# ebiggers/libdeflate

Hardware: NVIDIA H100
Metric: MB/s compress+decompress (batched 64 KiB chunks) (higher is better)
Workload: dtype u8

## Files before the change

### libdeflate_b200/csrc/deflate_lz_kernel.cuh

```cuda
#pragma once

#define LZ_THREADS   1024
#define LZ_WARPS     (LZ_THREADS / 32)
#define LZ_PASS      16384
#define LZ_BLOCK_PASSES 2
#define LZ_NWIN      (LZ_PASS / 32)
#define LZ_NSL_BITS  5
#define LZ_NSL       (1 << LZ_NSL_BITS)
#define LZ_SEG       16384
#define LZ_RING      65536
#define LZ_HASH_BITS 13
#define LZ_WIN       32768
#define LZ_LOOKAHEAD 512
#define LZ_MAX_DIST  (LZ_WIN - LZ_LOOKAHEAD)
#define LZ_TOKCAP    (LZ_BLOCK_PASSES * LZ_PASS + 64)
#define LZ_STAGE_WORDS 2048
#define LZ_TPT(gt)     ((gt) > 512 ? 1u : 2u)
#define LZ_GROUP_PARSE     {12, 10, 8, 8, 8, 5, 16, 16, 16}
#define LZ_GROUP_FLUSH     12
#define LZ_GROUP_HAND      10
#define LZ_GROUP_MIN_PARSE 4
#define LZ_GROUP_MIN_FLUSH 10
#define LZ_GROUP_MAX       28
#define LZ_BAR_P     1
#define LZ_BAR_S     2
#define LZ_BAR_H     3
#define LZ_PF        4
#define LZ_RUN_SHORT 16
#ifndef LZ_SPEC_ROUNDS
#define LZ_SPEC_ROUNDS 4
#endif
static_assert(LZ_SPEC_ROUNDS >= 1 && LZ_SPEC_ROUNDS <= 14, "round statistic buckets");
static_assert(LZ_GROUP_MIN_PARSE >= 1 && LZ_GROUP_MIN_FLUSH * 32 >= 320 && LZ_GROUP_MAX < LZ_WARPS, "group size bounds");
static_assert(LZ_GROUP_FLUSH >= LZ_GROUP_MIN_FLUSH && LZ_GROUP_FLUSH <= LZ_GROUP_MAX && LZ_GROUP_HAND >= LZ_GROUP_MIN_FLUSH &&
	      LZ_GROUP_HAND <= LZ_GROUP_MAX, "default group sizes");

#define LZ_SM_RING   0
#define LZ_SM_NEXT   (LZ_SM_RING + LZ_RING)
#define LZ_SM_HEAD   (LZ_SM_NEXT + 2 * 65536)
#define LZ_SM_R      (LZ_SM_HEAD + 2 * (1 << LZ_HASH_BITS))
#define LZ_SM_VIS    (LZ_SM_R)
#define LZ_SM_TOKOFF (LZ_SM_R + 4096)
#define LZ_SM_ENTRY  (LZ_SM_R + 8320)
#define LZ_SM_ESCAN  (LZ_SM_R + 9344)
#define LZ_SM_GEXIT  (LZ_SM_R + 9728)
#define LZ_SM_ITEMS  (LZ_SM_R + 12288)
#define LZ_SM_FREQ   (LZ_SM_ITEMS + 1024)
#define LZ_SM_LENS   (LZ_SM_FREQ + 4 * 320)
#define LZ_SM_CODES  (LZ_SM_LENS + 320)
#define LZ_SM_VARS   (LZ_SM_CODES + 2 * 320)
#define LZ_SM_BYTES  (LZ_SM_VARS + 256)

#define LZ_BLOCK_POS (LZ_BLOCK_PASSES * LZ_PASS)
#define LZ_OPT_K     8
#define LZ_DP_SEG    2048
#define LZ_GS_RES    0
#define LZ_GS_TOK    (LZ_GS_RES + 4 * LZ_BLOCK_POS)
#define LZ_GS_COST   (LZ_GS_TOK + 4 * LZ_TOKCAP)
#define LZ_GS_MLIST  (LZ_GS_COST + 4 * (LZ_BLOCK_POS + 320))
#define LZ_GS_BYTES  (LZ_GS_MLIST + 4 * LZ_BLOCK_POS * LZ_OPT_K)
#define LZ_FAR4_DIST  1024
#define LZ_COST_INF  0x3fffffu

struct lz_vars {
	unsigned long long mbar;
	u32 chunk;
	u32 tok_count;
	u32 parse_entry;
	u32 cost_dyn, cost_static;
	u32 hlit, hdist, hclen;
	u32 n_items;
	u32 run_counter;
	u32 min_len;
	u32 far4_dist;
	u32 used_lits[8];
	u32 carry;
	u32 nused_lit, nused_off;
	u32 huff_over;
	u32 obs_blk[8], obs_next[8];
	u32 end_block;
	u32 failed;
	u32 obit_lo, obit_hi;
	u32 blk_begin, blk_entry, blk_passes;
	u32 pre_lens_packed[3];
	u32 tma_phase;
	u32 dict, nonfinal;
	u32 spec_last;
	u32 spec_first;
	u32 prefetched;
	u32 nx_min_len, nx_far4;
};
static_assert(sizeof(lz_vars) <= 256, "lz_vars fits its shared-memory slot");

struct lz_params {
	int depth, nice, lazy;
	int opt_iters;
};

__device__ __forceinline__ lz_params lz_level_params(int level)
{
	switch (level) {
	case 1: return {2, 16, 0, 0};
	case 2: return {4, 24, 0, 0};
	case 3: return {8, 32, 0, 0};
	case 4: return {12, 48, 0, 0};
	case 5: return {12, 48, 1, 0};
	case 6: return {24, 96, 1, 0};
	case 7: return {48, 160, 1, 0};
	case 8: return {96, 258, 2, 0};
	case 9: return {200, 258, 2, 0};
	case 10: return {48, 96, 1, 2};
	case 11: return {96, 160, 1, 3};
	default: return {200, 258, 1, 5};
	}
}

__device__ __forceinline__ u32 lz_choose_min_len(u32 num_used_literals, u32 depth)
{
	u32 m;
	if (num_used_literals < 6) m = 9;
	else if (num_used_literals < 8) m = 8;
	else if (num_used_literals < 10) m = 7;
	else if (num_used_literals < 16) m = 6;
	else if (num_used_literals < 45) m = 5;
	else m = 4;
	if (depth < 16) {
		u32 cap = depth < 5 ? 4 : (depth < 10 ? 5 : 7);
		if (m > cap) m = cap;
	}
	return m;
}

__device__ __forceinline__ u32 lz_ld32(const u8 *ring, u32 pos)
{
	u32 a = pos & (LZ_RING - 1);
	const u32 *w = (const u32 *)ring;
	u32 lo = w[a >> 2];
	u32 hi = w[((a + 4) & (LZ_RING - 1)) >> 2];
	return __funnelshift_r(lo, hi, (a & 3) * 8);
}
__device__ __forceinline__ u32 lz_ld8(const u8 *ring, u32 pos) { return ring[pos & (LZ_RING - 1)]; }
__device__ __forceinline__ u32 lz_hash(u32 v) { return (v * 0x1E35A7BDu) >> (32 - LZ_HASH_BITS); }

__device__ __forceinline__ u32 lz_len_slot(u32 len)
{
	if (len < 11) return len - 3;
	if (len == 258) return 28;
	u32 l = len - 3;
	u32 eb = 29 - __clz(l);
	return 4 * eb + 4 + ((l >> eb) & 3);
}
__device__ __forceinline__ u32 lz_len_extra_bits(u32 slot) { return (slot < 8 || slot == 28) ? 0 : (slot - 4) >> 2; }
__device__ __forceinline__ u32 lz_len_base(u32 slot) { return slot < 8 ? 3 + slot : (slot == 28 ? 258 : 3 + ((4 + (slot & 3)) << ((slot - 4) >> 2))); }
__device__ __forceinline__ u32 lz_off_slot(u32 off)
{
	if (off < 5) return off - 1;
	u32 o = off - 1;
	u32 eb = 30 - __clz(o);
	return 2 * eb + 2 + ((o >> eb) & 1);
}
__device__ __forceinline__ u32 lz_off_extra_bits(u32 slot) { return slot < 4 ? 0 : (slot - 2) >> 1; }
__device__ __forceinline__ u32 lz_off_base(u32 slot) { return slot < 4 ? 1 + slot : 1 + ((2 + (slot & 1)) << ((slot - 2) >> 1)); }

#include "deflate_block.cuh"

__device__ __forceinline__ void lz_load_segment(const lz_group &g, u8 *sm, const u8 *in, u32 from, u32 to)
{
	u8 *ring = sm + LZ_SM_RING;
	lz_vars *v = (lz_vars *)(sm + LZ_SM_VARS);
	u32 len = to - from;
	u32 bulk = (((uintptr_t)(in + from) & 15) == 0) ? (len & ~15u) : 0;
	g.sync();
#ifndef LDB_EMU
	if (bulk) {
		u32 mbar = (u32)__cvta_generic_to_shared(&v->mbar);
		if (g.tid == 0) {
			u32 dst = (u32)__cvta_generic_to_shared(ring + (from & (LZ_RING - 1)));
			asm volatile("fence.proxy.async.shared::cta;" ::: "memory");
			asm volatile("mbarrier.arrive.expect_tx.shared::cta.b64 _, [%0], %1;" ::"r"(mbar), "r"(bulk) : "memory");
			asm volatile("cp.async.bulk.shared::cluster.global.mbarrier::complete_tx::bytes [%0], [%1], %2, [%3];"
				     ::"r"(dst), "l"(in + from), "r"(bulk), "r"(mbar) : "memory");
		}
		u32 phase = v->tma_phase;
		u32 done = 0;
		while (!done) {
			asm volatile("{\n\t.reg .pred p;\n\tmbarrier.try_wait.parity.shared::cta.b64 p, [%1], %2;\n\tselp.u32 %0, 1, 0, p;\n\t}"
				     : "=r"(done) : "r"(mbar), "r"(phase) : "memory");
		}
	}
#else
	for (u32 i = g.tid; i < bulk; i += g.gt) ring[(from + i) & (LZ_RING - 1)] = in[from + i];
#endif
	for (u32 i = bulk + g.tid; i < len; i += g.gt) ring[(from + i) & (LZ_RING - 1)] = in[from + i];
	g.sync();
	if (bulk && g.tid == 0) v->tma_phase ^= 1;
	g.sync();
}

#ifdef LZ_TIMING
#include <stdio.h>
#define LZ_TSLOTS 30
__device__ unsigned long long ldb_lz_timing[2][LZ_TSLOTS];
struct lz_clock {
	bool on, t0;
	long long tacc[LZ_TSLOTS] = {}, tlast = 0, tspan = 0, tsplit = 0, tbusy = 0, tjoin = 0;
	__device__ explicit lz_clock(u32 tid)
	{
		on = tid == 0 || tid == LZ_THREADS - 32;
		t0 = tid == 0;
		tlast = clock64();
	}
	__device__ void mark(int k) { if (on) { const long long t = clock64(); tacc[k] += t - tlast; tlast = t; } }
	__device__ void span_begin() { if (on) tspan = clock64(); }
	__device__ void span_end(int k) { if (on) tacc[k] += clock64() - tspan; }
	__device__ void split_begin() { if (on) tsplit = clock64(); }
	__device__ void split_busy() { if (t0) tbusy = clock64() - tsplit; }
	__device__ void join_begin() { if (on) tjoin = clock64(); }
	__device__ void split_end(bool split, int kind)
	{
		if (!split || !on) return;
		const long long t = clock64();
		tacc[18 + kind] += tbusy; tacc[21 + kind] += t - tjoin; tacc[24 + kind] += 1; tacc[27 + kind] += t - tsplit;
	}
	__device__ void commit() const
	{
		if (on)
			for (int k = 0; k < LZ_TSLOTS; k++) atomicAdd(&ldb_lz_timing[t0 ? 0 : 1][k], (unsigned long long)tacc[k]);
	}
};
#else
struct lz_clock {
	__device__ explicit lz_clock(u32) {}
	__device__ __forceinline__ void mark(int) {}
	__device__ __forceinline__ void span_begin() {}
	__device__ __forceinline__ void span_end(int) {}
	__device__ __forceinline__ void split_begin() {}
	__device__ __forceinline__ void split_busy() {}
	__device__ __forceinline__ void join_begin() {}
	__device__ __forceinline__ void split_end(bool, int) {}
	__device__ __forceinline__ void commit() const {}
};
#endif

#ifdef LZ_SPEC_STATS
__device__ unsigned long long ldb_lz_spec_rounds[16];
extern "C" __attribute__((visibility("default"))) void ldb_lz_spec_stats(unsigned long long *out, int reset)
{
#ifdef LDB_EMU
	for (int i = 0; i < 16; i++) { out[i] = ldb_lz_spec_rounds[i]; if (reset) ldb_lz_spec_rounds[i] = 0; }
#else
	unsigned long long z[16] = {};
	cudaDeviceSynchronize();
	cudaMemcpyFromSymbol(out, ldb_lz_spec_rounds, sizeof(z));
	if (reset) cudaMemcpyToSymbol(ldb_lz_spec_rounds, z, sizeof(z));
#endif
}
#endif

template <int NBITS>
__device__ __forceinline__ u32 lz_same_key_mask(u32 key, bool valid)
{
	u32 m = __ballot_sync(LDB_FULL_MASK, valid);
#pragma unroll
	for (int b = 0; b < NBITS; b++) {
		const u32 bal = __ballot_sync(LDB_FULL_MASK, (key >> b) & 1);
		m &= ((key >> b) & 1) ? bal : ~bal;
	}
	return m;
}

template <typename Decided>
__device__ __forceinline__ void lz_insert_pass_par(const lz_group &g, u8 *sm, u32 *cmat, u32 b0, u32 pend, u32 n,
						   bool decide, Decided decided, lz_clock &clk)
{
	const u8 *ring = sm + LZ_SM_RING;
	u16 *head = (u16 *)(sm + LZ_SM_HEAD);
	u16 *nextt = (u16 *)(sm + LZ_SM_NEXT);
	const u32 tid = g.tid, lane = g.lane, warp = g.warp, gw = g.gw;
	static_assert((LZ_WARPS * LZ_NSL + 2 * LZ_NSL) * 4 <= 8192, "count matrix fits the start of region R");
	u32 *sbase = cmat + LZ_WARPS * LZ_NSL, *stot = sbase + LZ_NSL;
	const u32 lt = (1u << lane) - 1;
	const u32 LB = (b0 + LZ_PASS) & 0xffff;
	const u32 ntiles = (pend - b0 + 31) >> 5, tpw = (ntiles + gw - 1) / gw;
	const u32 r0 = b0 + warp * tpw * 32;
	const u32 r1 = r0 + tpw * 32 < pend ? r0 + tpw * 32 : pend;
	for (u32 i = tid; i < LZ_WARPS * LZ_NSL + 2 * LZ_NSL; i += 32 * gw) cmat[i] = 0;
	g.sync();
	for (u32 p = r0 + lane; p < r1; p += 32) {
		const u32 hv = p + 4 <= n ? lz_hash(lz_ld32(ring, p)) : 0xffffu;
		nextt[p & 0xffff] = (u16)hv;
		if (hv != 0xffffu) atomicAdd(&cmat[warp * LZ_NSL + (hv >> (LZ_HASH_BITS - LZ_NSL_BITS))], 1u);
	}
	g.sync();
	clk.mark(12);
	if (decide && tid == 32 * (gw - 1)) decided();
	if (warp == 0) {
		u32 run = 0;
		if (lane < LZ_NSL)
			for (u32 w = 0; w < gw; w++) {
				const u32 c = cmat[w * LZ_NSL + lane];
				cmat[w * LZ_NSL + lane] = run;
				run += c;
			}
		u32 incl = run;
		for (int o2 = 1; o2 < LZ_NSL; o2 <<= 1) {
			const u32 t = __shfl_up_sync(LDB_FULL_MASK, incl, o2);
			if (lane >= (u32)o2) incl += t;
		}
		if (lane < LZ_NSL) { sbase[lane] = incl - run; stot[lane] = run; }
	}
	g.sync();
	for (u32 t = 0; t < tpw; t++) {
		const u32 p = r0 + 32 * t + lane;
		const u32 hv = p < r1 ? nextt[p & 0xffff] : 0xffffu;
		const bool valid = hv != 0xffffu;
		const u32 sl = hv >> (LZ_HASH_BITS - LZ_NSL_BITS);
		const u32 m = lz_same_key_mask<LZ_NSL_BITS>(sl, valid);
		const u32 cur = valid ? cmat[warp * LZ_NSL + sl] : 0;
		__syncwarp();
		if (valid) {
			nextt[LB + sbase[sl] + cur + __popc(m & lt)] = (u16)p;
			if ((m & lt) == 0) cmat[warp * LZ_NSL + sl] = cur + __popc(m);
		}
		__syncwarp();
	}
	g.sync();
	clk.mark(13);
	for (u32 s = warp; s < LZ_NSL; s += gw) {
		const u32 cnt = stot[s];
		const u16 *mylist = nextt + LB + sbase[s];
		u32 p16n = lane < cnt ? mylist[lane] : 0;
		u32 hn = lane < cnt ? nextt[p16n] : 0;
		for (u32 b = 0; b < cnt; b += 32) {
			const bool valid = b + lane < cnt;
			const u32 p16 = p16n;
			const u32 h = valid ? hn : 0;
			if (b + 32 + lane < cnt) {
				p16n = mylist[b + 32 + lane];
				hn = nextt[p16n];
			}
			const u32 old_head = valid ? head[h] : 0;
			const u32 m = lz_same_key_mask<LZ_HASH_BITS - LZ_NSL_BITS>(h, valid);
			const u32 below = m & lt;
			const u32 prev = __shfl_sync(LDB_FULL_MASK, p16, below ? 31 - __clz(below) : 0);
			if (valid) {
				nextt[p16] = (u16)(below ? prev : old_head);
				if ((m >> lane) == 1) head[h] = (u16)p16;
			}
			__syncwarp();
		}
	}
	g.sync();
}

__device__ __forceinline__ void lz_observe(const u8 *ring, u32 from, u32 to, u32 *obs, u32 tid, u32 lane, u32 nthreads)
{
	for (u32 wbase = from + 512 * (tid >> 5); wbase < to; wbase += 16 * nthreads) {
		const u32 base = wbase + 16 * lane;
		const uint4 q = *(const uint4 *)(ring + (base & (LZ_RING - 1)));
		const u32 w[4] = {q.x, q.y, q.z, q.w};
		u64 cnt = 0;
#pragma unroll
		for (int k = 0; k < 16; k++) {
			const u32 bv = (w[k >> 2] >> (8 * (k & 3))) & 0xff;
			if (base + k < to) cnt += (u64)1 << (8 * (((bv >> 5) & 6) | (bv & 1)));
		}
		u64 lo = cnt & 0x00ff00ff00ff00ffull, hi = (cnt >> 8) & 0x00ff00ff00ff00ffull;
		for (int o = 16; o > 0; o >>= 1) {
			lo += __shfl_xor_sync(LDB_FULL_MASK, lo, o);
			hi += __shfl_xor_sync(LDB_FULL_MASK, hi, o);
		}
		if (lane < 4) atomicAdd(&obs[2 * lane], (u32)(lo >> (16 * lane)) & 0xffff);
		else if (lane < 8) atomicAdd(&obs[2 * (lane - 4) + 1], (u32)(hi >> (16 * (lane - 4))) & 0xffff);
	}
}

__device__ __forceinline__ bool lz_should_end_block(const u32 *obs, const u32 *obs_new, u32 block_length)
{
	u32 n_old = 0, n_new = 0;
	for (int i = 0; i < 8; i++) { n_old += obs[i]; n_new += obs_new[i]; }
	if (!n_old || !n_new) return false;
	u64 total_delta = 0;
	for (int i = 0; i < 8; i++) {
		const u64 expected = (u64)obs[i] * n_new, actual = (u64)obs_new[i] * n_old;
		total_delta += actual > expected ? actual - expected : expected - actual;
	}
	const u64 cutoff = (u64)n_new * 200 / 512 * n_old;
	return total_delta + (u64)(block_length / 4096) * n_old >= cutoff;
}

__device__ __forceinline__ void lz_end_block_decide(lz_vars *v, u32 passes, u32 block_length)
{
	const bool end = passes == LZ_BLOCK_PASSES || lz_should_end_block(v->obs_blk, v->obs_next, block_length);
	v->end_block = end ? 1 : 0;
	for (int k = 0; k < 8; k++) {
		v->obs_blk[k] = end ? v->obs_next[k] : v->obs_blk[k] + v->obs_next[k];
		v->obs_next[k] = 0;
	}
}

__device__ __forceinline__ bool lz_stored_chunk(size_t n, size_t avail, int format, int level)
{
	const u32 overhead = ldb_wrap_bytes(format);
	return n <= (size_t)(55 - 4 * level) || n > 0x7fff0000u || (overhead && avail <= overhead);
}

#define LZ_DICT (PIECES ? v->dict : 0u)
#define LZ_NONFINAL (PIECES && v->nonfinal)

#include "deflate_parse.cuh"

template <bool PIECES>
__global__ void __launch_bounds__(LZ_THREADS, 1)
ldb_deflate_lz_kernel(ldb_deflate_args a)
{
	LDB_DYN_SMEM(sm);
	u8 *ring = sm + LZ_SM_RING;
	u16 *head = (u16 *)(sm + LZ_SM_HEAD);
	u16 *nextt = (u16 *)(sm + LZ_SM_NEXT);
	u32 *freq = (u32 *)(sm + LZ_SM_FREQ);
	lz_vars *v = (lz_vars *)(sm + LZ_SM_VARS);
	u8 *gs = a.scratch + 256 + (size_t)blockIdx.x * LZ_GS_BYTES;
	u32 *res = (u32 *)(gs + LZ_GS_RES);
	u32 *tokbuf = (u32 *)(gs + LZ_GS_TOK);
	u32 *costg = (u32 *)(gs + LZ_GS_COST);
	u32 *mlist = (u32 *)(gs + LZ_GS_MLIST);

	const u32 tid = threadIdx.x, lane = tid & 31, warp = tid >> 5;
	lz_clock clk(tid);
	const lz_params P = lz_level_params(a.level);
	const bool pipe = !P.opt_iters;
	const lz_group cta = lz_group_of(0, LZ_WARPS, LZ_BAR_P);

	if (tid == 0) {
		v->tma_phase = 0;
		v->prefetched = 0;
#ifndef LDB_EMU
		u32 mbar = (u32)__cvta_generic_to_shared(&v->mbar);
		asm volatile("mbarrier.init.shared::cta.b64 [%0], 1;" ::"r"(mbar) : "memory");
		asm volatile("fence.mbarrier_init.release.cluster;" ::: "memory");
#endif
	}
	__syncthreads();

	for (;;) {
		if (tid == 0 && !v->prefetched) v->chunk = atomicAdd(a.work_counter, 1u);
		__syncthreads();
		const size_t c = v->chunk;
		const bool pre = v->prefetched == 2;
		__syncthreads();
		if (tid == 0) v->prefetched = 0;
		if (c >= a.n) break;

		const u32 pflags = PIECES ? a.piece[c] : 0;
		const u32 dict = pflags & LDB_PIECE_DICT_MASK;
		const bool final_piece = !(pflags & LDB_PIECE_NONFINAL);
		const u8 *in = (const u8 *)a.in_ptrs[c];
		const size_t n64 = a.in_nbytes[c];
		lz_out o;
		o.out = (u8 *)a.out_ptrs[c];
		o.avail = a.out_avail[c];
		o.obit = 0;
		const u32 hdr_bytes = ldb_hdr_bytes(a.format);
		if (lz_stored_chunk(n64, o.avail, a.format, a.level)) {
			def_write_stored_chunk(a, c, tid, LZ_THREADS);
			continue;
		}
		const u32 n = (u32)n64 + dict;
		in -= dict;

		if (tid == 0) {
			if (pre) { v->min_len = v->nx_min_len; v->far4_dist = v->nx_far4; }
			else for (int k = 0; k < 8; k++) v->obs_next[k] = 0;
			v->failed = 0;
			v->parse_entry = dict;
			if (PIECES) { v->dict = dict; v->nonfinal = !final_piece; }
			v->tok_count = 0;
			u8 h[12] = {0, 0, 0, 0, 0, 0, 0, 0, 0, 0, 0, 0};
			def_write_header(h, a.format, a.level);
			u32 whole = hdr_bytes & ~3u;
			for (u32 i = 0; i < whole; i++) o.out[i] = h[i];
			u32 cw = 0;
			for (u32 i = whole; i < hdr_bytes; i++) cw |= (u32)h[i] << (8 * (i - whole));
			v->carry = cw;
		}
		for (u32 i = tid; i < 320; i += LZ_THREADS) freq[i] = 0;
		o.obit = (u64)hdr_bytes * 8;
		__syncthreads();

		u32 loaded_end = pre ? (n < 2 * LZ_PASS + 16 ? n : 2 * LZ_PASS + 16) : 0;
		lz_blockpos bp = {dict, dict, 0};

		const u32 npass = (n + LZ_PASS - 1) / LZ_PASS;
		const bool hand_on = pipe && !PIECES && (npass & 3) == 0;
		bool handed = false;
		for (u32 step = pre ? 1 : 0; step < npass + (pipe ? 1 : 0); step++) {
			const u32 b0 = step * LZ_PASS;
			const u32 pend = b0 + LZ_PASS < n ? b0 + LZ_PASS : n;
			clk.span_begin();
			size_t c1 = 0;
			u32 n1 = 0;
			bool beside = false;
			if (hand_on && step == npass) {
				c1 = v->chunk;
				if (c1 < a.n) {
					const size_t m64 = a.in_nbytes[c1];
					n1 = (u32)m64;
					beside = !lz_stored_chunk(m64, a.out_avail[c1], a.format, a.level);
				}
			}
			const u32 hw = a.pwarps[2];
			const bool sg = beside && warp >= hw;
			if (step < npass || sg) {
				const lz_group lg = lz_group_of(sg ? hw : 0, sg ? LZ_WARPS - hw : LZ_WARPS, LZ_BAR_S);
				const u8 *src = sg ? (const u8 *)a.in_ptrs[c1] : in;
				const u32 fn = sg ? n1 : n, fb0 = sg ? 0 : b0, fpend = sg ? (n1 < LZ_PASS ? n1 : LZ_PASS) : pend;
				if (sg) loaded_end = 0;
				if (lg.tid == 0) {
					v->run_counter = 0;
					if (hand_on && step + 1 == npass) { v->chunk = atomicAdd(a.work_counter, 1u); v->prefetched = 1; }
				}
				if (fb0 == 0)
					for (u32 i = lg.tid; i < (1u << LZ_HASH_BITS) / 2; i += lg.gt) ((u32 *)head)[i] = 0xffffffffu;
				lg.sync();
				{
					const u32 want = fpend + LZ_PASS + 16 < fn ? fpend + LZ_PASS + 16 : fn;
					while (loaded_end < want) {
						u32 room = LZ_RING - (loaded_end & (LZ_RING - 1));
						u32 to = loaded_end + (room < LZ_SEG ? room : LZ_SEG);
						if (to > want) to = want;
						lz_load_segment(lg, sm, src, loaded_end, to);
						loaded_end = to;
					}
				}
				if (fb0 == LZ_DICT) {
					if (lg.tid < 8) { v->used_lits[lg.tid] = 0; v->obs_blk[lg.tid] = 0; }
					lg.sync();
					lz_observe(ring, fb0, fpend, v->obs_blk, lg.tid, lane, lg.gt);
					const u32 own = fn - LZ_DICT, scan = own < 4096 ? own : 4096;
					for (u32 i = lg.tid; i < scan; i += lg.gt) {
						u32 bv = ring[(fb0 + i) & (LZ_RING - 1)];
						atomicOr(&v->used_lits[bv >> 5], 1u << (bv & 31));
					}
					lg.sync();
					if (lg.tid == 0) {
						u32 cnt = 0;
						for (int k = 0; k < 8; k++) cnt += __popc(v->used_lits[k]);
						(sg ? v->nx_min_len : v->min_len) = own < 512 ? 4 : lz_choose_min_len(cnt, (u32)P.depth);
						(sg ? v->nx_far4 : v->far4_dist) = cnt < 80 ? LZ_FAR4_DIST : LZ_WIN;
					}
					lg.sync();
				}
				clk.mark(0);
				u32 *cmat = sg ? (u32 *)(nextt + 2 * LZ_PASS) : (u32 *)(sm + LZ_SM_R);
				const bool decide = pipe && !sg && step > LZ_DICT / LZ_PASS;
				lz_insert_pass_par(lg, sm, cmat, fb0, fpend, fn, decide,
						   [&]() { lz_end_block_decide(v, bp.passes + 1, b0 - bp.begin); }, clk);
				clk.mark(3);
				if (step == 0) clk.span_end(17);
				if (sg) LDB_BAR_ARRIVE(LZ_BAR_H, LZ_THREADS);
			}
			const u32 gw = !pipe ? LZ_WARPS : step < npass ? (v->end_block ? a.pwarps[1] : a.pwarps[0]) : (beside ? hw : LZ_WARPS);
			const lz_group pg = lz_group_of(0, gw, LZ_BAR_P);
			if (!pipe) {
				if (PIECES && step < v->dict / LZ_PASS) continue;
				lz_search_all_pass(pg, sm, P, b0, pend, n, res, mlist, bp.passes * LZ_PASS);
				clk.mark(1);
				lz_parse_and_flush<PIECES>(pg, sm, P, a.format, in, n, res, tokbuf, costg, mlist, b0, pend, bp.passes * LZ_PASS,
							   nextt + ((b0 + LZ_PASS) & 0xffff), o, bp, clk);
			} else {
				clk.split_begin();
				if (tid < pg.gt && step > LZ_DICT / LZ_PASS) {
					const u32 kb0 = b0 - LZ_PASS;
					lz_parse_and_flush<PIECES>(pg, sm, P, a.format, in, n, res, tokbuf, costg, mlist, kb0,
								   kb0 + LZ_PASS < n ? kb0 + LZ_PASS : n, ((step - 1) & 1) * LZ_PASS,
								   nextt + ((kb0 + (beside ? 0 : 2 * LZ_PASS)) & 0xffff), o, bp, clk);
					if (beside) lz_finish(pg, sm, a, c, o, LZ_NONFINAL);
					clk.split_busy();
					if (beside) LDB_BAR_SYNC(LZ_BAR_H, LZ_THREADS);
				}
				if ((step < npass && (!PIECES || step >= v->dict / LZ_PASS)) || beside) {
					const u32 spend = beside ? (n1 < LZ_PASS ? n1 : LZ_PASS) : pend, snn = beside ? n1 : n;
					if (warp >= LZ_GROUP_MAX && spend < snn)
						lz_observe(ring, spend, spend + LZ_PASS < snn ? spend + LZ_PASS : snn, v->obs_next,
							   tid - 32 * LZ_GROUP_MAX, lane, LZ_THREADS - 32 * LZ_GROUP_MAX);
					lz_search_pass(sm, P, a.level, beside ? 0 : b0, spend, res + (beside ? 0 : (step & 1) * LZ_PASS), snn,
						       beside ? v->nx_min_len : v->min_len, beside ? v->nx_far4 : v->far4_dist, &v->run_counter);
				}
				clk.mark(1);
				if (tid == 0) lz_publish(v, bp, o);
				if (beside && tid == LZ_THREADS - 32) v->prefetched = 2;
			}
			clk.join_begin();
			__syncthreads();
			clk.mark(14);
			clk.split_end(pipe && step > LZ_DICT / LZ_PASS && (step < npass || beside), beside ? 2 : (v->blk_passes == 0 ? 1 : 0));
			if (step == npass) clk.span_end(16);
			if (beside) { handed = true; break; }
			if (v->failed) break;
			if (pipe) lz_adopt(v, bp, o);
		}
		if (handed) continue;
		__syncthreads();
		lz_finish(cta, sm, a, c, o, LZ_NONFINAL);
		__syncthreads();
		clk.mark(7);
	}
	clk.commit();
}

#ifdef LZ_TIMING
extern "C" __attribute__((visibility("default"))) void ldb_lz_timing_dump(void)
{
	unsigned long long h[2][LZ_TSLOTS], z[2][LZ_TSLOTS] = {};
	cudaDeviceSynchronize();
	cudaMemcpyFromSymbol(h, ldb_lz_timing, sizeof(h));
	cudaMemcpyToSymbol(ldb_lz_timing, z, sizeof(z));
	const char *names[18] = {"loads+first", "search", "parse e5", "insert: linking", "huffman", "precode", "cost+emit", "chunk pro/epilogue",
				 "parse e1 steps", "parse e2 walks", "parse e3 exit", "parse e4", "insert: hashing", "insert: slice lists", "wait at join", "",
				 "(span) last step", "(span) step 0 load+insert"};
	const char *who[2] = {"thread 0 (parse/flush group; levels 10-12: whole CTA)", "first thread of the last warp (search group)"};
	for (int g = 0; g < 2; g++) {
		unsigned long long tot = 0;
		for (int k = 0; k < 15; k++) tot += h[g][k];
		printf("  timing, clocked by %s:\n", who[g]);
		for (int k = 0; k < 18; k++)
			if (h[g][k]) printf("  timing %-26s %14llu cycles  %5.1f%%\n", names[k], h[g][k], 100.0 * (double)h[g][k] / (double)tot);
	}
	const char *kinds[3] = {"parse only", "parse + flush", "hand-over"};
	unsigned long long all_span = 0;
	for (int k = 0; k < 3; k++) all_span += h[1][27 + k];
	printf("  timing split steps       steps   span/step   p-busy/step  s-wait/step  p-wait/step  s-wait %%span  s-wait %%all-split\n");
	for (int k = 0; k < 3; k++) {
		const double ns = h[1][24 + k] ? (double)h[1][24 + k] : 1.0;
		printf("  timing %-15s %10llu %11.0f %13.0f %12.0f %12.0f %12.1f%% %12.1f%%\n", kinds[k], h[1][24 + k], h[1][27 + k] / ns,
		       h[0][18 + k] / ns, h[1][21 + k] / ns, h[0][21 + k] / ns,
		       h[1][27 + k] ? 100.0 * (double)h[1][21 + k] / (double)h[1][27 + k] : 0.0,
		       all_span ? 100.0 * (double)h[1][21 + k] / (double)all_span : 0.0);
	}
}
#endif

size_t ldb_deflate_scratch_bytes(const ldb_launch_cfg &cfg, size_t n)
{
	size_t ctas = n < (size_t)ldb_deflate_grid(cfg) ? n : (size_t)ldb_deflate_grid(cfg);
	return 256 + ctas * LZ_GS_BYTES;
}

static int ldb_launch_deflate_lz(const ldb_deflate_args &a, const ldb_launch_cfg &cfg, void *stream)
{
	LDB_CUDA_CHECK_RET(cudaFuncSetAttribute(a.piece ? ldb_deflate_lz_kernel<true> : ldb_deflate_lz_kernel<false>,
						cudaFuncAttributeMaxDynamicSharedMemorySize, LZ_SM_BYTES));
	ldb_deflate_args b = a;
	b.work_counter = (u32 *)a.scratch;
	ldb_deflate_groups(a.level, b.pwarps);
	LDB_CUDA_CHECK_RET(cudaMemsetAsync(b.work_counter, 0, sizeof(u32), (cudaStream_t)stream));
	size_t blocks = a.n < (size_t)ldb_deflate_grid(cfg) ? a.n : (size_t)ldb_deflate_grid(cfg);
	if (a.piece)
		LDB_LAUNCH(ldb_deflate_lz_kernel<true>, dim3((unsigned)blocks), dim3(LZ_THREADS), LZ_SM_BYTES, (cudaStream_t)stream, b);
	else
		LDB_LAUNCH(ldb_deflate_lz_kernel<false>, dim3((unsigned)blocks), dim3(LZ_THREADS), LZ_SM_BYTES, (cudaStream_t)stream, b);
	LDB_CUDA_CHECK_RET(cudaGetLastError());
	return 0;
}
```

### libdeflate_b200/csrc/deflate_parse.cuh

```cuda
#pragma once

__device__ __forceinline__ void lz_search(const u8 *ring, const u16 *nextt, u32 p, u32 n, int depth, u32 nice_level,
					   u32 &best_len, u32 &best_dist)
{
	const u32 max_len = n - p < 258 ? n - p : 258;
	const u32 nice = nice_level < max_len ? nice_level : max_len;
	if (best_len) {
		while (best_len < max_len && lz_ld8(ring, p + best_len) == lz_ld8(ring, p - best_dist + best_len)) best_len++;
	}
	if (best_len >= nice) return;
	const u32 cur = lz_ld32(ring, p);
	u32 tailo = best_len >= 4 ? best_len - 3 : 0;
	u32 tailv = tailo ? lz_ld32(ring, p + tailo) : cur;
	const u32 lim = p < LZ_MAX_DIST ? p : LZ_MAX_DIST;
	u32 cand = nextt[p & 0xffff];
	u32 prev_dist = 0;
	for (int d = 0; d < depth; d++) {
		const u32 dist = (p - cand) & 0xffff;
		if (dist - 1 >= lim || dist <= prev_dist) break;
		prev_dist = dist;
		const u32 cq = cand;
		cand = nextt[cq];
		if (lz_ld8(ring, cq + tailo + 3) != (tailv >> 24)) continue;
		if (lz_ld32(ring, cq + tailo) != tailv) continue;
		if (tailo && lz_ld32(ring, cq) != cur) continue;
		u32 len = 4;
		while (len + 4 <= max_len) {
			u32 x = lz_ld32(ring, p + len) ^ lz_ld32(ring, cq + len);
			if (x) { len += (__ffs(x) - 1) >> 3; goto extended; }
			len += 4;
		}
		while (len < max_len && lz_ld8(ring, p + len) == lz_ld8(ring, cq + len)) len++;
	extended:
		if (len > best_len) {
			best_len = len;
			best_dist = dist;
			if (len >= nice) break;
			tailo = len - 3;
			tailv = lz_ld32(ring, p + tailo);
		}
	}
}

__device__ __forceinline__ void lz_search_all(const u8 *ring, const u16 *nextt, u32 p, u32 n, int depth, u32 nice_level,
					       u32 *ml, u32 &best_len, u32 &best_dist)
{
	const u32 max_len = n - p < 258 ? n - p : 258;
	const u32 nice = nice_level < max_len ? nice_level : max_len;
	const u32 cur = lz_ld32(ring, p);
	u32 tailo = 0, tailv = cur, cnt = 0;
	best_len = 0;
	best_dist = 0;
	const u32 lim = p < LZ_MAX_DIST ? p : LZ_MAX_DIST;
	u32 cand = nextt[p & 0xffff];
	u32 prev_dist = 0;
	for (int d = 0; d < depth; d++) {
		const u32 dist = (p - cand) & 0xffff;
		if (dist - 1 >= lim || dist <= prev_dist) break;
		prev_dist = dist;
		const u32 cq = cand;
		cand = nextt[cq];
		if (lz_ld8(ring, cq + tailo + 3) != (tailv >> 24)) continue;
		if (lz_ld32(ring, cq + tailo) != tailv) continue;
		if (tailo && lz_ld32(ring, cq) != cur) continue;
		u32 len = 4;
		while (len + 4 <= max_len) {
			u32 x = lz_ld32(ring, p + len) ^ lz_ld32(ring, cq + len);
			if (x) { len += (__ffs(x) - 1) >> 3; goto extended; }
			len += 4;
		}
		while (len < max_len && lz_ld8(ring, p + len) == lz_ld8(ring, cq + len)) len++;
	extended:
		if (len > best_len) {
			best_len = len;
			best_dist = dist;
			ml[cnt < LZ_OPT_K ? cnt : LZ_OPT_K - 1] = (len << 16) | (dist - 1);
			cnt++;
			if (len >= nice) break;
			tailo = len - 3;
			tailv = lz_ld32(ring, p + tailo);
		}
	}
	for (u32 k = cnt; k < LZ_OPT_K; k++) ml[k] = 0;
}

__device__ void lz_dp_segment(const u8 *ring, const u32 *mlist, u32 *costg, u32 *res, const u8 *costtab,
			      u32 block_begin, u32 s0, u32 s1, u32 lane)
{
	const u8 *litc = costtab, *lenc = costtab + 256, *offc = costtab + 256 + 259;
	u32 wc = lane == 0 ? 0 : LZ_COST_INF;
	u32 i = s1;
	auto load_tile = [&](u32 top) -> u32 {
		u32 q = lane >> 3;
		if (top < q + 1 || top - 1 - q < s0) return 0;
		return mlist[(size_t)(top - 1 - q) * LZ_OPT_K + (lane & 7)];
	};
	u32 nxt = load_tile(i);
	while (i > s0) {
		const u32 curt = nxt;
		nxt = i >= 4 ? load_tile(i - 4) : 0;
#pragma unroll
		for (int q = 0; q < 4; q++) {
			if (i < (u32)q + 1 || i - 1 - q < s0) break;
			const u32 pos = i - 1 - q;
			u32 m[LZ_OPT_K];
#pragma unroll
			for (int j = 0; j < LZ_OPT_K; j++) m[j] = __shfl_sync(LDB_FULL_MASK, curt, q * 8 + j);
			u32 Lmax = 0;
#pragma unroll
			for (int j = 0; j < LZ_OPT_K; j++)
				if (m[j]) Lmax = m[j] >> 16;
			const u32 cap = s1 - pos;
			if (Lmax > cap) Lmax = cap;
			const u32 byte = ring[(block_begin + pos) & (LZ_RING - 1)];
			auto dist_for = [&](u32 L) -> u32 {
				u32 d = 0;
#pragma unroll
				for (int j = LZ_OPT_K - 1; j >= 0; j--)
					if (m[j] && (m[j] >> 16) >= L) d = (m[j] & 0xffff) + 1;
				return d;
			};
			u32 key;
			{
				const u32 L = lane + 1;
				u32 cand = LZ_COST_INF;
				if (lane == 0) cand = wc + litc[byte];
				else if (L >= 4 && L <= Lmax) cand = wc + lenc[L] + offc[lz_off_slot(dist_for(L))];
				if (cand > LZ_COST_INF) cand = LZ_COST_INF;
				key = (cand << 9) | (L - 1);
			}
			for (u32 base = 32; base < Lmax; base += 32) {
				const u32 L = base + lane + 1;
				if (L <= Lmax) {
					u32 c = pos + L == s1 ? 0 : costg[pos + L];
					u32 cand = c + lenc[L] + offc[lz_off_slot(dist_for(L))];
					if (cand > LZ_COST_INF) cand = LZ_COST_INF;
					u32 k2 = (cand << 9) | (L - 1);
					if (k2 < key) key = k2;
				}
			}
#pragma unroll
			for (int o = 16; o > 0; o >>= 1) {
				u32 other = __shfl_xor_sync(LDB_FULL_MASK, key, o);
				if (other < key) key = other;
			}
			const u32 C = key >> 9, bestL = (key & 511) + 1;
			if (lane == 0) {
				costg[pos] = C;
				if (bestL >= 3) {
					res[pos] = bestL | (((dist_for(bestL) - 1) | 0x8000u) << 16);
				} else {
					res[pos] = 0;
				}
			}
			const u32 t = __shfl_up_sync(LDB_FULL_MASK, wc, 1);
			wc = lane == 0 ? C : t;
		}
		i = i >= 4 ? i - 4 : 0;
	}
	__syncwarp();
}
__device__ __forceinline__ void lz_search_pass(u8 *sm, const lz_params &P, int level, u32 b0, u32 pend, u32 *rs, u32 nn,
					       u32 min_len, u32 far4, u32 *run_counter)
{
	const u8 *ring = sm + LZ_SM_RING;
	const u16 *nextt = (const u16 *)(sm + LZ_SM_NEXT);
	const u32 run_len = level >= 7 ? 32 : LZ_RUN_SHORT;
	u32 i = 0, i_end = 0;
	u32 pL = 0, pD = 0;
	u32 pending = 0;
	for (;;) {
		if (i >= i_end || b0 + i >= pend) {
			const u32 r = atomicAdd(run_counter, 1u);
			i = r * run_len;
			if (b0 + i >= pend || i >= LZ_PASS) break;
			i_end = i + run_len;
			pending = 0;
		}
		const u32 p = b0 + i;
		u32 L = 0, D = 0;
		if (p + 4 <= nn) {
			if (pending) { L = pL - pending >= 4 ? pL - pending : 0; D = pD; }
			lz_search(ring, nextt, p, nn, P.depth >> pending, (u32)P.nice, L, D);
		}
		rs[i] = L ? L | ((D - 1) << 16) : 0;
		u32 mpos, mL, mD;
		if (pending) {
			const int margin = pending == 1 ? 2 : 6;
			if (L >= pL && 4 * ((int)L - (int)pL) + ((int)(31 - __clz((int)pD)) - (int)(31 - __clz((int)D))) > margin) {
				mpos = i; mL = L >= (u32)P.nice ? L : 0; mD = D;
				if (!mL) { pL = L; pD = D; }
				pending = mL == 0 ? 1 : 0;
			} else if (pending == 1 && P.lazy == 2 && i + 1 < i_end && b0 + i + 1 < pend) {
				pending = 2;
				mpos = i; mL = 0; mD = 0;
			} else {
				mpos = i - pending; mL = pL; mD = pD;
				pending = 0;
			}
		} else if (L >= min_len && !(L == 4 && D > far4)) {
			if (P.lazy && L < (u32)P.nice && i + 1 < i_end && b0 + i + 1 < pend) {
				pending = 1; pL = L; pD = D;
				mpos = i; mL = 0; mD = 0;
			} else {
				mpos = i; mL = L; mD = D;
			}
		} else {
			mpos = i; mL = 0; mD = 0;
		}
		if (mL) {
			u32 stop = mpos + mL < i_end ? mpos + mL : i_end;
			if (b0 + stop > pend) stop = pend - b0;
			u32 mend = b0 + mpos + mL;
			for (u32 k = i + 1; k < stop; k++) {
				const u32 pk = b0 + k;
				if (mL == 258)
					while (mend < nn && mend - pk < 258 && lz_ld8(ring, mend) == lz_ld8(ring, mend - mD)) mend++;
				u32 lk = mend - pk;
				rs[k] = lk >= 4 ? lk | ((mD - 1) << 16) : 0;
			}
			i = mpos + mL;
		} else {
			i++;
		}
	}
}

__device__ __forceinline__ void lz_search_all_pass(const lz_group &g, u8 *sm, const lz_params &P, u32 b0, u32 pend, u32 n,
						   u32 *res, u32 *mlist, u32 aoff)
{
	const u8 *ring = sm + LZ_SM_RING;
	const u16 *nextt = (const u16 *)(sm + LZ_SM_NEXT);
	u32 *rs = res + aoff;
	for (u32 i = g.tid; b0 + i < pend; i += g.gt) {
		const u32 p = b0 + i;
		u32 L = 0, D = 0;
		u32 *ml = mlist + (size_t)(aoff + i) * LZ_OPT_K;
		if (p + 4 <= n) {
			lz_search_all(ring, nextt, p, n, P.depth, (u32)P.nice, ml, L, D);
		} else {
			for (u32 k = 0; k < LZ_OPT_K; k++) ml[k] = 0;
		}
		rs[i] = L ? L | ((D - 1) << 16) : 0;
	}
	g.sync();
}


__device__ __forceinline__ void lz_parse_steps(const lz_group &g, u8 *sm, const lz_params &P, const u32 *res, u32 aoff, u32 pb0,
					       u32 ppend, bool forced, u16 *exitt, lz_clock &clk)
{
	const lz_vars *v = (const lz_vars *)(sm + LZ_SM_VARS);
	const u32 lane = g.lane;
	const u32 nwin = (ppend - pb0 + 31) >> 5;
	const u32 min_len = v->min_len, far4 = v->far4_dist;
	const u32 G = (nwin + g.gw - 1) / g.gw;
	const u32 wbeg = g.warp * G, wend = wbeg + G < nwin ? wbeg + G : nwin;
	auto res_load = [&](u32 w) -> u32 {
		const u32 i = w * 32 + lane;
		return w < nwin && pb0 + i < ppend ? res[aoff + i] : 0;
	};
	u32 q[LZ_PF];
#pragma unroll
	for (int k = 0; k < LZ_PF; k++) q[k] = res_load(wbeg + k);
	for (u32 w = wbeg; w < wend; w++) {
		u32 i = w * 32 + lane;
		u32 p = pb0 + i;
		const u32 W0 = q[0], nx = q[1];
#pragma unroll
		for (int k = 0; k + 1 < LZ_PF; k++) q[k] = q[k + 1];
		q[LZ_PF - 1] = res_load(w + LZ_PF);
		const u32 nx0 = __shfl_sync(LDB_FULL_MASK, nx, 0), nx1 = __shfl_sync(LDB_FULL_MASK, nx, 1);
		const u32 nb = __shfl_down_sync(LDB_FULL_MASK, W0, 1), W1 = lane == 31 ? nx0 : nb;
		const u32 nb2 = __shfl_down_sync(LDB_FULL_MASK, W1, 1), W2 = lane == 31 ? nx1 : nb2;
		const u32 L0 = W0 & 0xffff, O0 = ((W0 >> 16) & 0x7fff) + 1, L1 = W1 & 0xffff, O1 = ((W1 >> 16) & 0x7fff) + 1;
		bool is_match = forced ? ((W0 >> 31) && p < ppend) : (L0 >= min_len && p < ppend && !(L0 == 4 && O0 > far4));
		if (!forced && is_match && P.lazy && p + 1 < ppend) {
			if (L1 >= L0 && L0 < (u32)P.nice &&
			    4 * ((int)L1 - (int)L0) + ((int)(31 - __clz((int)O0)) - (int)(31 - __clz((int)O1))) > 2)
				is_match = false;
			if (P.lazy == 2 && is_match && p + 2 < ppend) {
				const u32 L2 = W2 & 0xffff, O2 = ((W2 >> 16) & 0x7fff) + 1;
				if (L2 >= L0 && L0 < (u32)P.nice &&
				    4 * ((int)L2 - (int)L0) + ((int)(31 - __clz((int)O0)) - (int)(31 - __clz((int)O2))) > 6)
					is_match = false;
			}
		}
		exitt[w * 32 + (lane ^ (w & 31))] = (u16)(is_match ? L0 : 1);
	}
	g.sync();
	clk.mark(8);
}

__device__ __forceinline__ u32 lz_walk(const u16 *exitt, u32 w, u32 k, u32 stop, u32 &m)
{
	const u16 *st = exitt + w * 32;
	const u32 sw = w & 31;
	m = 0;
	while (k < 32 && !((stop >> k) & 1)) {
		m |= 1u << k;
		k += st[k ^ sw];
	}
	return k;
}

__device__ __forceinline__ u32 lz_rewalk(const u16 *exitt, u32 *vis, u32 w, u32 oe, u32 ne, u32 ox)
{
	u32 m = 0;
	if (ne != 0xff) {
		const u32 old = oe != 0xff ? vis[w] : 0;
		const u32 k = lz_walk(exitt, w, ne, old, m);
		if (k < 32) m |= old & ~((1u << k) - 1);
		else ox = w * 32 + k;
	}
	vis[w] = m;
	return ox;
}

__device__ __forceinline__ u32 lz_derive(u32 w, u32 pe, u32 we, const u8 *e, const u16 *x)
{
	if (w <= we) return w < we ? 0xff : (pe & 31);
	for (u32 d = 1; d <= 9 && d <= w - we; d++) {
		if (e[w - d] == 0xff) continue;
		const u32 xw = x[w - d] >> 5;
		return xw == w ? (x[w - d] & 31) : (xw > w ? 0xff : 0xfe);
	}
	return 0xfe;
}

__device__ __forceinline__ void lz_parse_walks(const lz_group &g, u8 *sm, u32 pb0, u32 ppend, const u16 *exitt, lz_clock &clk)
{
	lz_vars *v = (lz_vars *)(sm + LZ_SM_VARS);
	u32 *vis = (u32 *)(sm + LZ_SM_VIS);
	u8 *entryt = sm + LZ_SM_ENTRY;
	u16 *gexit = (u16 *)(sm + LZ_SM_GEXIT);
	const u32 tid = g.tid;
	const u32 nwin = (ppend - pb0 + 31) >> 5;
	const u32 pe = v->parse_entry - pb0, we = pe >> 5;
	u8 *ent = entryt;
	u16 *wx = gexit;
	for (u32 w = tid; w < nwin; w += g.gt) {
		const u32 e0 = w < we ? 0xff : (w == we ? (pe & 31) : 0);
		ent[w] = (u8)e0;
		wx[w] = (u16)lz_rewalk(exitt, vis, w, 0xff, e0, 0);
	}
	if (tid == 0) { v->spec_last = 0; v->spec_first = 0xffffu; }
	g.sync();
	u32 r = 1;
	for (;; r++) {
		const u8 *pent = ent;
		const u16 *pwx = wx;
		ent = entryt + (r & 1) * LZ_NWIN;
		wx = gexit + (r & 1) * LZ_NWIN;
		bool changed = false;
		for (u32 w = tid; w < nwin; w += g.gt) {
			const u32 oe = pent[w], ox = pwx[w];
			u32 ne = lz_derive(w, pe, we, pent, pwx);
			if (ne == 0xfe) ne = oe;
			u32 nx = ox;
			if (ne != oe) {
				nx = lz_rewalk(exitt, vis, w, oe, ne, ox);
				changed = true;
				if (r == LZ_SPEC_ROUNDS) atomicMin(&v->spec_first, w);
			}
			ent[w] = (u8)ne;
			wx[w] = (u16)nx;
		}
		if (changed) v->spec_last = r;
		g.sync();
		if (v->spec_last < r) break;
		if (r == LZ_SPEC_ROUNDS) {
			if (tid == 0) {
				u32 w = v->spec_first, pos = 0;
				while (w > we && ent[w] == 0xff) w--;
				pos = wx[w];
				for (w++; w < nwin; w++) {
					u32 e = 0xff, m = 0;
					if ((pos >> 5) == w) {
						e = pos & 31;
						pos = w * 32 + lz_walk(exitt, w, e, 0, m);
						wx[w] = (u16)pos;
					}
					ent[w] = (u8)e;
					vis[w] = m;
				}
			}
			r++;
			break;
		}
	}
	clk.mark(9);
	if (tid == 0) {
#ifdef LZ_SPEC_STATS
		atomicAdd(&ldb_lz_spec_rounds[r], 1ull);
#endif
		u32 fin = pe;
		for (u32 w = nwin; w > we;) {
			w--;
			if (ent[w] != 0xff) { fin = wx[w]; break; }
		}
		fin += pb0;
		v->parse_entry = fin < ppend ? ppend : fin;
		const u32 part = (ppend - pb0) & 31;
		if (part) vis[nwin - 1] &= (1u << part) - 1;
	}
	g.sync();
	clk.mark(10);
}

__device__ __forceinline__ void lz_parse_tokens(const lz_group &g, u8 *sm, const u32 *res, u32 aoff, u32 *tokbuf, u32 pb0, u32 ppend,
						u32 n, const u16 *exitt, lz_clock &clk)
{
	lz_vars *v = (lz_vars *)(sm + LZ_SM_VARS);
	const u8 *ring = sm + LZ_SM_RING;
	const u32 *vis = (const u32 *)(sm + LZ_SM_VIS);
	u32 *tokoff = (u32 *)(sm + LZ_SM_TOKOFF);
	u32 *freq = (u32 *)(sm + LZ_SM_FREQ);
	const u32 lane = g.lane;
	const u32 nwin = (ppend - pb0 + 31) >> 5;
	if (g.warp == 0) {
		u32 run = 0;
		for (u32 w0 = 0; w0 < nwin; w0 += 32) {
			const u32 w = w0 + lane;
			const u32 c = w < nwin ? (u32)__popc(vis[w]) : 0;
			const u32 incl = lz_warp_incl_scan(c, lane);
			if (w < nwin) tokoff[w] = run + incl - c;
			run += __shfl_sync(LDB_FULL_MASK, incl, 31);
		}
		if (lane == 0) tokoff[LZ_NWIN] = run;
	}
	g.sync();
	clk.mark(11);
	const u32 G = (nwin + g.gw - 1) / g.gw;
	const u32 wbeg = g.warp * G, wend = wbeg + G < nwin ? wbeg + G : nwin;
	const u32 tbase = v->tok_count;
	auto e5_load = [&](u32 w) -> u32 {
		return w < nwin && ((vis[w] >> lane) & 1) ? res[aoff + w * 32 + lane] : 0;
	};
	u32 q[LZ_PF];
#pragma unroll
	for (int k = 0; k < LZ_PF; k++) q[k] = e5_load(wbeg + k);
	for (u32 w = wbeg; w < wend; w++) {
		const u32 V = vis[w], ro = q[0] >> 16;
		const u32 len = q[0] & 0xffff;
#pragma unroll
		for (int k = 0; k + 1 < LZ_PF; k++) q[k] = q[k + 1];
		q[LZ_PF - 1] = e5_load(w + LZ_PF);
		if (!V) continue;
		u32 i = w * 32 + lane;
		if ((V >> lane) & 1) {
			u32 idx = tbase + tokoff[w] + __popc(V & ((1u << lane) - 1));
			u32 off = (ro & 0x7fff) + 1;
			if (exitt[w * 32 + (lane ^ (w & 31))] > 1 && len >= 3 && len <= 258 && off <= pb0 + i && pb0 + i + len <= n) {
				tokbuf[idx] = 0x80000000u | ((len - 3) << 15) | (off - 1);
				atomicAdd(&freq[257 + lz_len_slot(len)], 1u);
				atomicAdd(&freq[288 + lz_off_slot(off)], 1u);
			} else {
				u32 bv = lz_ld8(ring, pb0 + i);
				tokbuf[idx] = bv;
				atomicAdd(&freq[bv], 1u);
			}
		}
	}
	g.sync();
	if (g.tid == 0) v->tok_count = tbase + tokoff[LZ_NWIN];
	g.sync();
}

__device__ __forceinline__ void lz_parse_pass(const lz_group &g, u8 *sm, const lz_params &P, const u32 *res, u32 aoff, u32 *tokbuf,
					      u32 pb0, u32 ppend, u32 n, bool forced, u16 *exitt, lz_clock &clk)
{
	lz_parse_steps(g, sm, P, res, aoff, pb0, ppend, forced, exitt, clk);
	lz_parse_walks(g, sm, pb0, ppend, exitt, clk);
	lz_parse_tokens(g, sm, res, aoff, tokbuf, pb0, ppend, n, exitt, clk);
}

__device__ __forceinline__ void lz_optimize_block(const lz_group &g, u8 *sm, const lz_params &P, u32 block_begin, u32 block_entry,
						  u32 block_end, u32 npass, u32 *res, u32 *tokbuf, u32 *costg, const u32 *mlist,
						  u32 n, lz_clock &clk)
{
	lz_vars *v = (lz_vars *)(sm + LZ_SM_VARS);
	const u8 *ring = sm + LZ_SM_RING;
	u16 *nextt = (u16 *)(sm + LZ_SM_NEXT);
	u32 *freq = (u32 *)(sm + LZ_SM_FREQ);
	const u8 *lens = sm + LZ_SM_LENS;
	u8 *costtab = sm + LZ_SM_ITEMS;
	for (int it = 0; it < P.opt_iters; it++) {
		lz_build_codes(g, sm);
		for (u32 k = g.tid; k < 256 + 259 + 32; k += g.gt) {
			u32 c;
			if (k < 256) {
				c = lens[k] ? lens[k] : 13;
			} else if (k < 256 + 259) {
				u32 len = k - 256;
				if (len < 3) c = 255;
				else { u32 sl = lz_len_slot(len); c = (lens[257 + sl] ? lens[257 + sl] : 13) + lz_len_extra_bits(sl); }
			} else {
				u32 sl = k - 256 - 259;
				c = (lens[288 + sl] ? lens[288 + sl] : 10) + lz_off_extra_bits(sl);
			}
			costtab[k] = (u8)c;
		}
		g.sync();
		{
			const u32 rel_entry = block_entry - block_begin;
			const u32 blen_pos = block_end - block_begin;
			for (u32 seg = g.warp; seg * LZ_DP_SEG < blen_pos; seg += g.gw) {
				u32 s0 = seg * LZ_DP_SEG, s1 = s0 + LZ_DP_SEG < blen_pos ? s0 + LZ_DP_SEG : blen_pos;
				if (s0 < rel_entry) s0 = rel_entry;
				if (s0 >= s1) continue;
				lz_dp_segment(ring, mlist, costg, res, costtab, block_begin, s0, s1, g.lane);
			}
		}
		g.sync();
		for (u32 k = g.tid; k < 320; k += g.gt) freq[k] = 0;
		if (g.tid == 0) { v->tok_count = 0; v->parse_entry = block_entry; }
		g.sync();
		for (u32 pp = 0; pp < npass; pp++) {
			u32 pb0 = block_begin + pp * LZ_PASS;
			u32 ppend = pb0 + LZ_PASS < block_end ? pb0 + LZ_PASS : block_end;
			lz_parse_pass(g, sm, P, res, pp * LZ_PASS, tokbuf, pb0, ppend, n, true, nextt + ((block_begin + npass * LZ_PASS) & 0xffff), clk);
		}
	}
}

struct lz_blockpos {
	u32 begin, entry, passes;
};

__device__ __forceinline__ void lz_publish(lz_vars *v, const lz_blockpos &bp, const lz_out &o)
{
	v->obit_lo = (u32)o.obit; v->obit_hi = (u32)(o.obit >> 32);
	v->blk_begin = bp.begin; v->blk_entry = bp.entry; v->blk_passes = bp.passes;
}
__device__ __forceinline__ void lz_adopt(const lz_vars *v, lz_blockpos &bp, lz_out &o)
{
	o.obit = v->obit_lo | ((u64)v->obit_hi << 32);
	bp.begin = v->blk_begin; bp.entry = v->blk_entry; bp.passes = v->blk_passes;
}

template <bool PIECES>
__device__ __forceinline__ void lz_parse_and_flush(const lz_group &g, u8 *sm, const lz_params &P, int format, const u8 *in, u32 n,
						   u32 *res, u32 *tokbuf, u32 *costg, const u32 *mlist, u32 b0, u32 pend, u32 aoff,
						   u16 *exitt, lz_out &o, lz_blockpos &bp, lz_clock &clk)
{
	lz_vars *v = (lz_vars *)(sm + LZ_SM_VARS);
	const u8 *ring = sm + LZ_SM_RING;
	u32 *freq = (u32 *)(sm + LZ_SM_FREQ);
	u32 *stage = (u32 *)(sm + LZ_SM_R);
	const bool last = pend >= n;
	lz_parse_pass(g, sm, P, res, aoff, tokbuf, b0, pend, n, false, exitt, clk);
	clk.mark(2);
	bp.passes++;
	if (!last) {
		if (P.opt_iters) {
			if (g.tid < 8) v->obs_next[g.tid] = 0;
			g.sync();
			lz_observe(ring, pend, pend + LZ_PASS < n ? pend + LZ_PASS : n, v->obs_next, g.tid, g.lane, g.gt);
			g.sync();
			if (g.tid == 0) lz_end_block_decide(v, bp.passes, pend - bp.begin);
			g.sync();
		}
		if (!v->end_block) return;
	}
	const u32 npass_block = bp.passes;
	bp.passes = 0;
	const u32 block_end = pend;
	lz_optimize_block(g, sm, P, bp.begin, bp.entry, block_end, npass_block, res, tokbuf, costg, mlist, n, clk);
	clk.mark(7);
	lz_build_codes(g, sm);
	clk.mark(4);
	lz_precode(g, sm);
	clk.mark(5);
	const u32 blen = (v->parse_entry < n ? v->parse_entry : n) - bp.entry;
	const u32 btype = lz_block_choose(g, sm, o, blen, last ? (LZ_NONFINAL ? 5 : ldb_trl_bytes(format)) : 0);
	if (btype == LZ_NOFIT) return;
	lz_stage_reset(g, stage, o, &v->carry);
	if (btype == DEFLATE_BLOCKTYPE_STORED) lz_emit_stored(g, sm, o, in + bp.entry, blen, last && !LZ_NONFINAL);
	else lz_emit_huffman(g, sm, o, tokbuf, v->tok_count, btype, last && !LZ_NONFINAL);
	g.sync();
	if (g.tid == 0) v->carry = stage[0];
	clk.mark(6);
	bp.begin = block_end;
	bp.entry = v->parse_entry;
	for (u32 i = g.tid; i < 320; i += g.gt) freq[i] = 0;
	if (g.tid == 0) v->tok_count = 0;
	g.sync();
}
```

Before: 16380.

## Add ring guard band and unmasked 8-byte match-length comparisons

Extends the shared-memory ring buffer with a 512-byte guard that mirrors the first bytes after each load. Match search can then read past the wrap point without masking every index. Match extension now compares 8 bytes per iteration through a new lz_match_len helper, and the bytes after the current position are preloaded once per search instead of once per candidate. The extra copy into the guard costs one more pass and grows the shared-memory footprint, and the code is only correct if the guard is kept in sync with the ring.

```diff
diff --git a/libdeflate_b200/csrc/deflate_lz_kernel.cuh b/libdeflate_b200/csrc/deflate_lz_kernel.cuh
--- a/libdeflate_b200/csrc/deflate_lz_kernel.cuh
+++ b/libdeflate_b200/csrc/deflate_lz_kernel.cuh
@@ -9,6 +9,7 @@
 #define LZ_NSL       (1 << LZ_NSL_BITS)
 #define LZ_SEG       16384
 #define LZ_RING      65536
+#define LZ_RING_GUARD 512
 #define LZ_HASH_BITS 13
 #define LZ_WIN       32768
 #define LZ_LOOKAHEAD 512
@@ -36,7 +37,7 @@
 	      LZ_GROUP_HAND <= LZ_GROUP_MAX, "default group sizes");
 
 #define LZ_SM_RING   0
-#define LZ_SM_NEXT   (LZ_SM_RING + LZ_RING)
+#define LZ_SM_NEXT   (LZ_SM_RING + LZ_RING + LZ_RING_GUARD)
 #define LZ_SM_HEAD   (LZ_SM_NEXT + 2 * 65536)
 #define LZ_SM_R      (LZ_SM_HEAD + 2 * (1 << LZ_HASH_BITS))
 #define LZ_SM_VIS    (LZ_SM_R)
@@ -50,6 +51,9 @@
 #define LZ_SM_CODES  (LZ_SM_LENS + 320)
 #define LZ_SM_VARS   (LZ_SM_CODES + 2 * 320)
 #define LZ_SM_BYTES  (LZ_SM_VARS + 256)
+static_assert(LZ_SM_BYTES <= 232448, "the layout fits the opt-in shared memory of one sm_90 CTA");
+static_assert(LZ_RING_GUARD % 16 == 0 && LZ_RING_GUARD >= 258 + 16, "the guard keeps the layout 16-byte aligned and "
+	      "covers a 258-byte match read 8 bytes at a time (lz_match_len)");
 
 #define LZ_BLOCK_POS (LZ_BLOCK_PASSES * LZ_PASS)
 #define LZ_OPT_K     8
@@ -140,6 +144,34 @@
 	return __funnelshift_r(lo, hi, (a & 3) * 8);
 }
 __device__ __forceinline__ u32 lz_ld8(const u8 *ring, u32 pos) { return ring[pos & (LZ_RING - 1)]; }
+__device__ __forceinline__ u32 lz_ld32u(const u8 *ring, u32 a)
+{
+	const u32 *w = (const u32 *)ring + (a >> 2);
+	return __funnelshift_r(w[0], w[1], (a & 3) * 8);
+}
+__device__ __forceinline__ u32 lz_match_len(const u8 *ring, u32 a, u32 b, u32 len, u32 max_len)
+{
+	if (len >= max_len) return len;
+	const u32 *wa = (const u32 *)ring + ((a + len) >> 2), *wb = (const u32 *)ring + ((b + len) >> 2);
+	const u32 sa = ((a + len) & 3) * 8, sb = ((b + len) & 3) * 8;
+	u32 a0 = wa[0], b0 = wb[0];
+	for (;;) {
+		const u32 a1 = wa[1], a2 = wa[2], b1 = wb[1], b2 = wb[2];
+		const u32 x0 = __funnelshift_r(a0, a1, sa) ^ __funnelshift_r(b0, b1, sb);
+		const u32 x1 = __funnelshift_r(a1, a2, sa) ^ __funnelshift_r(b1, b2, sb);
+		if (x0 | x1) {
+			len += x0 ? (__ffs(x0) - 1) >> 3 : 4 + ((__ffs(x1) - 1) >> 3);
+			break;
+		}
+		len += 8;
+		if (len >= max_len) break;
+		wa += 2;
+		wb += 2;
+		a0 = a2;
+		b0 = b2;
+	}
+	return len < max_len ? len : max_len;
+}
 __device__ __forceinline__ u32 lz_hash(u32 v) { return (v * 0x1E35A7BDu) >> (32 - LZ_HASH_BITS); }
 
 __device__ __forceinline__ u32 lz_len_slot(u32 len)
@@ -194,6 +226,8 @@
 	for (u32 i = bulk + g.tid; i < len; i += g.gt) ring[(from + i) & (LZ_RING - 1)] = in[from + i];
 	g.sync();
 	if (bulk && g.tid == 0) v->tma_phase ^= 1;
+	const u32 lo = from & (LZ_RING - 1), hi = lo + len < LZ_RING_GUARD ? lo + len : LZ_RING_GUARD;
+	for (u32 i = lo + g.tid; i < hi; i += g.gt) ring[LZ_RING + i] = ring[i];
 	g.sync();
 }
 
diff --git a/libdeflate_b200/csrc/deflate_parse.cuh b/libdeflate_b200/csrc/deflate_parse.cuh
--- a/libdeflate_b200/csrc/deflate_parse.cuh
+++ b/libdeflate_b200/csrc/deflate_parse.cuh
@@ -5,15 +5,15 @@
 {
 	const u32 max_len = n - p < 258 ? n - p : 258;
 	const u32 nice = nice_level < max_len ? nice_level : max_len;
-	if (best_len) {
-		while (best_len < max_len && lz_ld8(ring, p + best_len) == lz_ld8(ring, p - best_dist + best_len)) best_len++;
-	}
+	const u32 pa = p & (LZ_RING - 1);
+	if (best_len) best_len = lz_match_len(ring, pa, (p - best_dist) & (LZ_RING - 1), best_len, max_len);
 	if (best_len >= nice) return;
-	const u32 cur = lz_ld32(ring, p);
+	const u32 *pw = (const u32 *)ring + (pa >> 2), ps = (pa & 3) * 8, w1 = pw[1], w2 = pw[2];
+	const u32 cur = __funnelshift_r(pw[0], w1, ps), pe0 = __funnelshift_r(w1, w2, ps), pe1 = __funnelshift_r(w2, pw[3], ps);
 	u32 tailo = best_len >= 4 ? best_len - 3 : 0;
-	u32 tailv = tailo ? lz_ld32(ring, p + tailo) : cur;
+	u32 tailv = tailo ? lz_ld32u(ring, pa + tailo) : cur;
 	const u32 lim = p < LZ_MAX_DIST ? p : LZ_MAX_DIST;
-	u32 cand = nextt[p & 0xffff];
+	u32 cand = nextt[pa];
 	u32 prev_dist = 0;
 	for (int d = 0; d < depth; d++) {
 		const u32 dist = (p - cand) & 0xffff;
@@ -21,23 +21,23 @@
 		prev_dist = dist;
 		const u32 cq = cand;
 		cand = nextt[cq];
-		if (lz_ld8(ring, cq + tailo + 3) != (tailv >> 24)) continue;
-		if (lz_ld32(ring, cq + tailo) != tailv) continue;
-		if (tailo && lz_ld32(ring, cq) != cur) continue;
-		u32 len = 4;
-		while (len + 4 <= max_len) {
-			u32 x = lz_ld32(ring, p + len) ^ lz_ld32(ring, cq + len);
-			if (x) { len += (__ffs(x) - 1) >> 3; goto extended; }
-			len += 4;
-		}
-		while (len < max_len && lz_ld8(ring, p + len) == lz_ld8(ring, cq + len)) len++;
-	extended:
+		if (ring[cq + tailo + 3] != (tailv >> 24)) continue;
+		if (lz_ld32u(ring, cq + tailo) != tailv) continue;
+		if (tailo && lz_ld32u(ring, cq) != cur) continue;
+		u32 len;
+		{
+			const u32 x0 = pe0 ^ lz_ld32u(ring, cq + 4), x1 = pe1 ^ lz_ld32u(ring, cq + 8);
+			if (x0) len = 4 + ((__ffs(x0) - 1) >> 3);
+			else if (x1) len = 8 + ((__ffs(x1) - 1) >> 3);
+			else len = lz_match_len(ring, pa, cq, 12, max_len);
+			if (len > max_len) len = max_len;
+		}
 		if (len > best_len) {
 			best_len = len;
 			best_dist = dist;
 			if (len >= nice) break;
 			tailo = len - 3;
-			tailv = lz_ld32(ring, p + tailo);
+			tailv = lz_ld32u(ring, pa + tailo);
 		}
 	}
 }
@@ -47,12 +47,14 @@
 {
 	const u32 max_len = n - p < 258 ? n - p : 258;
 	const u32 nice = nice_level < max_len ? nice_level : max_len;
-	const u32 cur = lz_ld32(ring, p);
+	const u32 pa = p & (LZ_RING - 1);
+	const u32 *pw = (const u32 *)ring + (pa >> 2), ps = (pa & 3) * 8, w1 = pw[1], w2 = pw[2];
+	const u32 cur = __funnelshift_r(pw[0], w1, ps), pe0 = __funnelshift_r(w1, w2, ps), pe1 = __funnelshift_r(w2, pw[3], ps);
 	u32 tailo = 0, tailv = cur, cnt = 0;
 	best_len = 0;
 	best_dist = 0;
 	const u32 lim = p < LZ_MAX_DIST ? p : LZ_MAX_DIST;
-	u32 cand = nextt[p & 0xffff];
+	u32 cand = nextt[pa];
 	u32 prev_dist = 0;
 	for (int d = 0; d < depth; d++) {
 		const u32 dist = (p - cand) & 0xffff;
@@ -60,17 +62,17 @@
 		prev_dist = dist;
 		const u32 cq = cand;
 		cand = nextt[cq];
-		if (lz_ld8(ring, cq + tailo + 3) != (tailv >> 24)) continue;
-		if (lz_ld32(ring, cq + tailo) != tailv) continue;
-		if (tailo && lz_ld32(ring, cq) != cur) continue;
-		u32 len = 4;
-		while (len + 4 <= max_len) {
-			u32 x = lz_ld32(ring, p + len) ^ lz_ld32(ring, cq + len);
-			if (x) { len += (__ffs(x) - 1) >> 3; goto extended; }
-			len += 4;
-		}
-		while (len < max_len && lz_ld8(ring, p + len) == lz_ld8(ring, cq + len)) len++;
-	extended:
+		if (ring[cq + tailo + 3] != (tailv >> 24)) continue;
+		if (lz_ld32u(ring, cq + tailo) != tailv) continue;
+		if (tailo && lz_ld32u(ring, cq) != cur) continue;
+		u32 len;
+		{
+			const u32 x0 = pe0 ^ lz_ld32u(ring, cq + 4), x1 = pe1 ^ lz_ld32u(ring, cq + 8);
+			if (x0) len = 4 + ((__ffs(x0) - 1) >> 3);
+			else if (x1) len = 8 + ((__ffs(x1) - 1) >> 3);
+			else len = lz_match_len(ring, pa, cq, 12, max_len);
+			if (len > max_len) len = max_len;
+		}
 		if (len > best_len) {
 			best_len = len;
 			best_dist = dist;
@@ -78,7 +80,7 @@
 			cnt++;
 			if (len >= nice) break;
 			tailo = len - 3;
-			tailv = lz_ld32(ring, p + tailo);
+			tailv = lz_ld32u(ring, pa + tailo);
 		}
 	}
 	for (u32 k = cnt; k < LZ_OPT_K; k++) ml[k] = 0;
@@ -214,8 +216,10 @@
 			u32 mend = b0 + mpos + mL;
 			for (u32 k = i + 1; k < stop; k++) {
 				const u32 pk = b0 + k;
-				if (mL == 258)
-					while (mend < nn && mend - pk < 258 && lz_ld8(ring, mend) == lz_ld8(ring, mend - mD)) mend++;
+				if (mL == 258 && mend < nn && mend - pk < 258) {
+					const u32 cap = nn - pk < 258 ? nn - pk : 258;
+					mend = pk + lz_match_len(ring, pk & (LZ_RING - 1), (pk - mD) & (LZ_RING - 1), mend - pk, cap);
+				}
 				u32 lk = mend - pk;
 				rs[k] = lk >= 4 ? lk | ((mD - 1) << 16) : 0;
 			}
```

Measured after the change: 16960, median of 6. 1.04x the previous value.
